# dusk-network/plonk_gadgets

Measured on AMD Instinct MI355X. Metric: gadget constraints/sec (range_check 256-bit), higher is better.
Workload: dtype u64x4 (BLS12-381 scalar, Montgomery limbs)

## Files before the change

### plonk_gadgets_amd/csrc/capi.hip

```cpp
#include "../../include/plonk_gadgets_hip.h"

#include <hip/hip_runtime.h>

#include <algorithm>
#include <cassert>
#include <cstdio>
#include <cstdlib>
#include <cstring>
#include <initializer_list>
#include <memory>
#include <new>
#include <functional>
#include <string>
#include <type_traits>
#include <utility>
#include <vector>

#include "emit.hpp"
#include "fr.hpp"
#include "range_gadgets.hpp"
#include "scalar_gadgets.hpp"
#include "composer.hpp"
#include "permutation.hpp"
#include "materialize.hpp"
// ... 191 lines not shown
#define PG_MIX_EARLY_TILES 1
#endif
#ifndef PG_INV_LANES_PER_CU
#define PG_INV_LANES_PER_CU 256
#endif
#ifndef PG_INV_MAX_PER_LANE
#define PG_INV_MAX_PER_LANE 32
#endif

pg_status launch_mix(pg_engine *e, const pg::ScalarMixArgs &A, const pg_columns *c, uint64_t batch, uint64_t gate_base,
                     uint64_t var_base, uint64_t zero_var, const uint64_t *row_off, const uint64_t *var_off, hipStream_t st,
                     const pg::MixPlan *planned, bool values_only = false) {
    using GD = pg::ScalarMixGD;
    PG_TRY(ensure_inv_scratch(e, batch));
    const uint64_t waves_wanted = (uint64_t)e->num_cus * 4 * 2;
    uint64_t ipl = (batch + waves_wanted * 32 - 1) / (waves_wanted * 32);
    if (ipl < 1) ipl = 1;
    if (ipl > pg::kMixMaxIpl) ipl = pg::kMixMaxIpl;
    const uint64_t waves = (batch + 32 * ipl - 1) / (32 * ipl);
    pg::EmitOut V = make_out(c, batch, GD::W, gate_base, var_base, zero_var, row_off, var_off);
    pg::EmitOut R = make_out(c, batch, GD::kRowsW, gate_base, var_base, zero_var, row_off, var_off);
    const uint64_t span = (uint64_t)pg::kMixWaves * 32 * ipl;
    if (!values_only && ipl >= 8 && span <= 0xffffffffull) {
        V.early_span = R.early_span = (uint32_t)span;
        V.early_tiles = R.early_tiles = PG_MIX_EARLY_TILES;
    }
    const uint32_t max_blocks = (uint32_t)e->num_cus * PG_GRID_BLOCKS_PER_CU;
    const dim3 grid(R.tiles < max_blocks ? R.tiles : max_blocks), vgrid((uint32_t)((waves + pg::kMixWaves - 1) / pg::kMixWaves));
    const dim3 vblock(pg::kMixWaves * 64);
    uint4 *const prefix = e->d_prefix.as<uint4>(), *sink = prefix + e->inv_elems * 4 + 4 * 32 * 32 * 8;
    if (planned) {
        pg::MixPlan P = *planned;
        P.nwaves = vgrid.x;
        hipLaunchKernelGGL(pg::scalar_mix_vars_kernel<true>, vgrid, vblock, 0, st, A, V, (uint32_t)ipl, prefix, sink, P);
    } else
        hipLaunchKernelGGL(pg::scalar_mix_vars_kernel<false>, vgrid, vblock, 0, st, A, V, (uint32_t)ipl, prefix, sink,
                           pg::MixPlan{});
    if (values_only) {
        PG_HIP_TRY(hipGetLastError());
        return PG_OK;
    }
    hipLaunchKernelGGL(pg::rows_periodic_kernel<GD>, grid, dim3(pg::kThreads), 0, st, A, R);
    hipLaunchKernelGGL((pg::emit_kernel<GD, pg::EMIT_ROWS>), grid, dim3(pg::kThreads), 0, st, A, R);
    PG_HIP_TRY(hipGetLastError());
    return PG_OK;
}

template <class GD> struct ValuesMode { static constexpr bool ok = !pg::Split<GD>::ok; };

template <class GD>
pg_status launch(pg_engine *e, const typename GD::Args &A, const pg_columns *c, uint64_t batch, uint64_t gate_base,
                 uint64_t var_base, uint64_t zero_var, const uint64_t *row_off, const uint64_t *var_off, void *stream,
                 const pg::MixPlan *planned = nullptr, bool values_only = false, uint32_t stride_rows = 0) {
    if ((batch + GD::W - 1) / GD::W > 0xffffffffull) return fail(PG_ERR_INVALID_ARGUMENT, "batch too large for one call");
    if (stride_rows && (batch > 0xffffffffull || pg::Split<GD>::ok || GD::kRagged))
        return fail(PG_ERR_INVALID_ARGUMENT, "a row stride is for uniform one-launch gadgets of at most 2^32 - 1 items");
    hipStream_t st = static_cast<hipStream_t>(stream);
    PG_TRY(enter_stream(e, st));
    StreamScope scope{e, st};
    if constexpr (pg::Split<GD>::ok) {
        return launch_mix(e, A, c, batch, gate_base, var_base, zero_var, row_off, var_off, st, planned, values_only);
    } else {
        pg::EmitOut O = make_out(c, batch, GD::W, gate_base, var_base, zero_var, row_off, var_off);
        if (stride_rows) {
            O.stride_rows = stride_rows;
            O.tiles = (uint32_t)batch;
        }
        bool side = false;
        SideJoin join{e, st};
        if constexpr (GD::kInv > 0) {
            constexpr int GRP = GD::kInvGroup;
            const uint64_t elems = batch * GD::kInv;
            PG_TRY(ensure_inv_scratch(e, elems));
            const uint64_t lanes_wanted = (uint64_t)e->num_cus * PG_INV_LANES_PER_CU;
            uint64_t per_lane = (elems + lanes_wanted - 1) / lanes_wanted;
            if (per_lane < 1) per_lane = 1;
            if (per_lane > PG_INV_MAX_PER_LANE) per_lane = PG_INV_MAX_PER_LANE;
            const uint64_t groups = (per_lane + GRP - 1) / GRP;
            const uint64_t lanes = (elems + groups * GRP - 1) / (groups * GRP);
            const uint32_t blocks = (uint32_t)((lanes + pg::kThreads - 1) / pg::kThreads);
            side = elems >= 2048 && elems < (1ull << 18);
            hipStream_t inv_st = st;
            if (side) {
                PG_HIP_TRY(hipEventRecord(e->ev_fork.get(), st));
                PG_HIP_TRY(hipStreamWaitEvent(e->side.get(), e->ev_fork.get(), 0));
                join.forked = true;
                inv_st = e->side.get();
            }
            if constexpr (pg::InvDense<GD>::ok) {
                O.inv_dense = e->d_prefix.as<uint4>();
                O.inv_elems = elems;
                O.inv_in_place = side;
            }
            hipLaunchKernelGGL((pg::batch_invert_kernel<GD, GRP>), dim3(blocks), dim3(pg::kThreads), 0, inv_st, A, O, elems,
                               (uint32_t)groups, e->d_prefix.as<uint4>());
            PG_HIP_TRY(hipGetLastError());
            if (side) PG_HIP_TRY(hipEventRecord(e->ev_inv.get(), e->side.get()));
        }
        const uint32_t max_blocks = (uint32_t)e->num_cus * (values_only ? PG_GRID_BLOCKS_PER_CU : PG_EMIT_GRID_BLOCKS_PER_CU);
        const dim3 egrid(O.tiles < max_blocks ? O.tiles : max_blocks);
        if (values_only) {
            if constexpr (ValuesMode<GD>::ok) hipLaunchKernelGGL((pg::emit_kernel<GD, pg::EMIT_VALUES>), egrid, dim3(pg::kThreads), 0, st, A, O);
            else return fail(PG_ERR_INVALID_ARGUMENT, "this gadget has no values-only emission");
        } else {
            hipLaunchKernelGGL(pg::emit_kernel<GD>, egrid, dim3(pg::kThreads), 0, st, A, O);
        }
        PG_HIP_TRY(hipGetLastError());
        if (side) {
            PG_HIP_TRY(hipStreamWaitEvent(st, e->ev_inv.get(), 0));
            join.joined = true;
        }
        return PG_OK;
    }
}

pg_status scalar_args(const pg_variable *a_var, const pg_scalar *a_val, const pg_variable *b_var,
// ... 1138 lines not shown
```

### plonk_gadgets_amd/csrc/emit.hpp

```cpp
#pragma once

#include <type_traits>

#include "fr.hpp"

namespace pg {

constexpr int kThreads = 256;

union FrVec {
    Fr f;
    uint4 v[2];
};

struct EmitOut {
    uint4 *q[5];
    uint64_t *w[3];
    uint4 *vars;
    uint64_t gate_base, var_base;
    uint64_t zero_var;
    const uint64_t *row_off;
    const uint64_t *var_off;
    uint64_t batch;
    uint32_t tiles;
    uint32_t stride_rows;
    const uint4 *inv_dense;
    uint64_t inv_elems;
    uint32_t inv_in_place;
    uint32_t early_span, early_tiles;
};
__device__ __forceinline__ bool early_rows_candidate(const EmitOut &O, uint64_t w0, uint32_t Wt, uint32_t W, uint64_t &s0, uint64_t &s1) {
    s0 = s1 = 0;
    if (!O.early_tiles || Wt != W) return false;
    s0 = w0 - w0 % O.early_span;
    s1 = s0 + O.early_span < O.batch ? s0 + O.early_span : O.batch;
    return (w0 - s0) / W < O.early_tiles;
}

__device__ __forceinline__ void fetch_inverse(const EmitOut &O, uint64_t s, void *rec_fr) {
    uint4 *z = reinterpret_cast<uint4 *>(rec_fr);
    z[0] = O.inv_dense[s];
    z[1] = O.inv_dense[O.inv_elems + s];
}

enum : uint32_t { T_ZERO = 0, T_ONE = 1, T_NEG1 = 2, T_QC_A = 3, T_QC_B = 4, T_POW = 8 };
constexpr int kTableEntries = 8 + 256;

typedef unsigned int pg_u32x4 __attribute__((ext_vector_type(4)));

__device__ __forceinline__ void store16(uint4 *p, uint4 v) {
#if defined(PG_NT_STORES)
    pg_u32x4 t = {v.x, v.y, v.z, v.w};
    __builtin_nontemporal_store(t, reinterpret_cast<pg_u32x4 *>(p));
#else
    *p = v;
#endif
}

__device__ __forceinline__ void lds_barrier() {
#if defined(PG_FULL_BARRIERS)
    __syncthreads();
#else
    asm volatile("s_waitcnt lgkmcnt(0)\n\ts_barrier" ::: "memory");
#endif
}

__device__ __forceinline__ uint64_t uniform64(uint64_t x) {
    return (uint64_t)(uint32_t)__builtin_amdgcn_readfirstlane((int)(uint32_t)x) |
           (uint64_t)(uint32_t)__builtin_amdgcn_readfirstlane((int)(uint32_t)(x >> 32)) << 32;
}

__device__ __forceinline__ Fr lds_fr(const uint4 *table, uint32_t id) {
    FrVec t;
    t.v[0] = table[2 * id];
    t.v[1] = table[2 * id + 1];
    return t.f;
}

__device__ __forceinline__ void fill_common_table(uint4 *table, const uint4 *pow2, uint32_t tid, uint32_t entries) {
    for (uint32_t e = tid; e < entries; e += kThreads) {
        FrVec t;
        t.f = fr_zero();
        if (e == T_ONE) t.f = fr_one();
        else if (e == T_NEG1) t.f = fr_neg_one();
        else if (e >= T_POW && pow2) { t.v[0] = pow2[(e - T_POW) * 2]; t.v[1] = pow2[(e - T_POW) * 2 + 1]; }
        if (e != T_QC_A && e != T_QC_B) {
            table[2 * e] = t.v[0];
            table[2 * e + 1] = t.v[1];
        }
    }
}

template <bool SMALL_ITEMS, uint32_t UNI>
__device__ __forceinline__ uint32_t find_item(const uint32_t *off, uint32_t Wt, uint32_t r, uint32_t it, bool uniform) {
    if constexpr (UNI != 0) {
        if (uniform) return r / UNI;
    }
    if constexpr (SMALL_ITEMS) {
// ... 22 lines not shown
struct Periodic {
    static constexpr bool ok = false;
};
template <class GD>
struct Periodic<GD, std::void_t<decltype(GD::kPeriodic)>> {
    static constexpr bool ok = GD::kPeriodic;
};
constexpr uint32_t periodic_wire_lanes(uint32_t R) {
    uint32_t L = 256;
    while ((2 * L) % R) L--;
    return L;
}

#ifndef PG_EMIT_WAVES_PER_SIMD
#define PG_EMIT_WAVES_PER_SIMD 1
#endif

enum EmitMode : int { EMIT_ALL = 0, EMIT_STRUCTURE = 1, EMIT_ROWS = 2, EMIT_VALUES = 3 };

template <class GD, class = void>
struct Split {
    static constexpr bool ok = false;
};
template <class GD>
struct Split<GD, std::void_t<decltype(GD::kSplit)>> {
    static constexpr bool ok = GD::kSplit;
};
template <class GD, class = void>
struct RegionVars {
    static constexpr bool ok = false;
};
template <class GD>
struct RegionVars<GD, std::void_t<decltype(GD::kRegionVars)>> {
    static constexpr bool ok = GD::kRegionVars;
};
template <class GD, class = void>
struct InvDense {
    static constexpr bool ok = false;
};
template <class GD>
struct InvDense<GD, std::void_t<decltype(GD::kInvDense)>> {
    static constexpr bool ok = GD::kInvDense;
};
template <class GD, int MODE>
struct EmitShape {
    using Rec = typename GD::ItemRec;
    static constexpr int W = GD::W;
};
template <class GD>
struct EmitShape<GD, EMIT_ROWS> {
    using Rec = typename GD::RowRec;
    static constexpr int W = GD::kRowsW;
};

constexpr uint32_t kRegionLead = 8, kRegionStage = (kRegionLead + 256 + 16) / 8 * 9;

template <class GD, int MODE = EMIT_ALL>
__global__ __launch_bounds__(kThreads, PG_EMIT_WAVES_PER_SIMD) void emit_kernel(const typename GD::Args A, const EmitOut O) {
    static_assert(MODE != EMIT_STRUCTURE || !(GD::kRagged || GD::kRecInRows), "rows of this gadget depend on its inputs");
    constexpr bool kVars = MODE == EMIT_ALL || MODE == EMIT_VALUES;
    constexpr bool kRows = MODE != EMIT_VALUES;
    constexpr int W = EmitShape<GD, MODE>::W;
    using Rec = typename EmitShape<GD, MODE>::Rec;
    constexpr uint32_t kTable = GD::kUsePow2 ? kTableEntries : T_POW;
    __shared__ uint4 s_table[kTable * 2];
    __shared__ Rec s_item[W];
    __shared__ uint32_t s_roff[W + 1], s_voff[W + 1];

    const uint32_t tid = threadIdx.x;
    {
        const uint4 *p2 = nullptr;
        if constexpr (GD::kUsePow2) p2 = GD::pow2(A);
        fill_common_table(s_table, p2, tid, kTable);
    }
    GD::fill_table(A, s_table, tid);
    lds_barrier();

    for (uint32_t t = blockIdx.x; t < O.tiles; t += gridDim.x) {
#if defined(PG_XCD_REMAP)
        const uint32_t q8 = O.tiles >> 3, r8 = O.tiles & 7, x = t & 7, k = t >> 3;
        const uint32_t tile = x * q8 + (x < r8 ? x : r8) + k;
#elif defined(PG_TILE_SPREAD)
        const uint32_t qs = O.tiles / PG_TILE_SPREAD, rs = O.tiles % PG_TILE_SPREAD, x = t % PG_TILE_SPREAD, k = t / PG_TILE_SPREAD;
        const uint32_t tile = x * qs + (x < rs ? x : rs) + k;
#else
        const uint32_t tile = t;
#endif
        const uint64_t w0 = O.stride_rows ? (uint64_t)tile : (uint64_t)tile * W;
        const uint32_t Wt = O.stride_rows ? 1u : (uint32_t)((O.batch - w0) < (uint64_t)W ? (O.batch - w0) : (uint64_t)W);
        if constexpr (MODE == EMIT_ROWS && Periodic<GD>::ok) {
            if (O.row_off[w0 + Wt] - O.row_off[w0] == (uint64_t)Wt * UniformShape<GD>::rows) continue;
        }
        uint64_t row0, var0;
        uint32_t G = 0, V = 0;
        uint64_t my_r = 0, my_v = 0, tail_r = 0, tail_v = 0;
        if constexpr (GD::kRagged) {
            row0 = O.row_off[w0];
            var0 = O.var_off[w0];
            if (tid <= Wt) {
                my_r = O.row_off[w0 + tid];
                my_v = O.var_off[w0 + tid];
            }
            if constexpr (W == kThreads) {
                if (tid == 0) {
                    tail_r = O.row_off[w0 + Wt];
                    tail_v = O.var_off[w0 + Wt];
                }
            }
        } else {
            G = GD::rows_per_item(A);
            V = GD::vars_per_item(A);
            row0 = w0 * (O.stride_rows ? O.stride_rows : G);
            var0 = w0 * V;
        }

        if constexpr ((GD::kRagged || GD::kRecInRows) && MODE != EMIT_STRUCTURE) {
            for (uint32_t i = tid; i < Wt; i += kThreads) GD::item_rows(A, O, w0 + i, s_table, s_item[i]);
        }
        if constexpr (GD::kRagged) {
            if (tid <= Wt) {
                s_roff[tid] = (uint32_t)(my_r - row0);
                s_voff[tid] = (uint32_t)(my_v - var0);
            }
            if constexpr (W == kThreads) {
                if (tid == 0) {
                    s_roff[Wt] = (uint32_t)(tail_r - row0);
                    s_voff[Wt] = (uint32_t)(tail_v - var0);
                }
            }
        }
        if constexpr (GD::kRagged || GD::kRecInRows) lds_barrier();
// ... 44 lines not shown
#if defined(PG_UNALIGNED_SWEEPS)
                const uint32_t pmis = 0;
#else
                const uint32_t pmis = (uint32_t)(((reinterpret_cast<uintptr_t>(col) - 8 * shift) >> 4) & 7u);
#endif
                uint32_t it = 0;
                for (uint32_t pv = tid < pmis ? tid + kThreads : tid; pv < pairs + pmis; pv += kThreads) {
                    const uint32_t p = pv - pmis;
                    const int64_t r0 = (int64_t)2 * p - shift;
                    uint64_t val[2];
#pragma unroll
                    for (int k = 0; k < 2; k++) {
                        const int64_t r = r0 + k;
                        uint32_t rr = r < 0 ? 0u : (uint32_t)r;
                        if (rr >= total_rows) rr = total_rows - 1;
                        uint32_t j, vo;
                        if constexpr (GD::kRagged) {
                            it = find_item<W >= 64, kUniR>(s_roff, Wt, rr, it, uni_rows);
                            j = uni_rows ? rr - it * kUniR : rr - s_roff[it];
                            vo = (uni_rows && uni_vars) ? it * kUniV : s_voff[it];
                        } else {
                            it = rr / G;
                            j = rr - it * G;
                            vo = it * V;
                        }
                        uint64_t out[3];
                        GD::wires(A, O, s_item[it], w0 + it, O.var_base + var0 + vo, j, out);
                        val[k] = out[c];
                    }
                    if (r0 >= 0 && r0 + 1 < (int64_t)total_rows) {
                        store16(reinterpret_cast<uint4 *>(col + r0),
                                make_uint4((uint32_t)val[0], (uint32_t)(val[0] >> 32), (uint32_t)val[1],
                                           (uint32_t)(val[1] >> 32)));
                    } else {
                        if (r0 >= 0) col[r0] = val[0];
                        if (r0 + 1 < (int64_t)total_rows) col[r0 + 1] = val[1];
                    }
                }
            }
        }

        lds_barrier();

        if constexpr (kVars) {
            const bool inv_here = InvDense<GD>::ok && !O.inv_in_place;
#if defined(PG_UNALIGNED_SWEEPS)
            const uint32_t smis = 0;
#else
            const uint32_t smis = (uint32_t)((reinterpret_cast<uintptr_t>(O.vars + var0 * 2) >> 5) & 3u);
#endif
#if !defined(PG_VAR_SWEEP_SINGLE)
            if constexpr (RegionVars<GD>::ok && MODE == EMIT_VALUES) {
                __shared__ uint4 s_reg[4 * kRegionStage];
                const uint32_t wave = tid >> 6, lane = tid & 63;
                uint4 *wp = s_reg + wave * kRegionStage;
                constexpr uint32_t B2 = 2 * GD::kBlocks;
                const uint32_t units = Wt * B2;
                const uint32_t tile_mis = (uint32_t)((reinterpret_cast<uintptr_t>(O.vars + var0 * 2) >> 5) & 3u);
                for (uint32_t q = wave; q < units; q += kThreads / 64) {
                    const uint32_t it = q / B2, r = q - it * B2, b = r >> 1;
                    const uint32_t kind = (r + (GD::kBlocks == 2 ? it : it >> 1)) & 1;
                    const Rec &R = s_item[it];
                    const auto &Bk = GD::region_block(R, b);
                    const uint32_t n = GD::region_n(A, R);
                    const uint32_t count = kind ? (n + 1 < 256 ? n + 1 : 256) : 256;
                    uint32_t vitem, vend;
                    if constexpr (GD::kRagged) {
                        vitem = uni_vars ? it * kUniV : s_voff[it];
                        vend = uni_vars ? vitem + kUniV : s_voff[it + 1];
                    } else {
                        vitem = it * V;
                        vend = vitem + V;
                    }
                    const uint32_t kfirst = GD::region_k(A, R, b, kind ? 257 : 1);
                    const uint32_t mis0 = (tile_mis + vitem) & 3u;
                    uint32_t ks, ke;
                    if (kind == 0) {
                        ks = b == 0 ? 0 : kfirst;
                        if (it != 0 || b != 0) ks += (4u - ((mis0 + ks) & 3u)) & 3u;
                        ke = kfirst + 256;
                        ke -= (mis0 + ke) & 3u;
                    } else {
                        ks = kfirst - ((mis0 + kfirst) & 3u);
                        ke = b + 1 < GD::kBlocks ? GD::region_k(A, R, b + 1, 1) : vend - vitem;
                        if (it + 1 != Wt || b + 1 < GD::kBlocks) ke += (4u - ((mis0 + ke) & 3u)) & 3u;
                    }
                    const uint32_t h_end = (count - 1) >> 7;
                    uint32_t hole = ~0u;
                    if (!inv_here)
                        for (uint32_t k = kfirst + count; k < ke && k < vend - vitem; k++)
                            if (GD::is_inv_slot(A, R, k)) hole = k;
                    FrVec v[4];
                    const uint32_t i0 = 4 * lane;
                    if (kind == 0) {
#pragma unroll
                        for (int t = 0; t < 4; t++) v[t].f = raw_bit(Bk.Tc, i0 + t) ? fr_one() : fr_zero();
                    } else {
                        v[0].f = fr_zero();
                        if (i0 && i0 < count) v[0].f = fr_to_mont(raw_low_bits(Bk.Tc, i0));
#pragma unroll
                        for (int t = 1; t < 4; t++) {
                            v[t].f = v[t - 1].f;
                            if (i0 + t < count && raw_bit(Bk.Tc, i0 + t - 1)) {
                                FrVec p;
                                p.v[0] = s_table[2 * (T_POW + i0 + t - 1)];
                                p.v[1] = s_table[2 * (T_POW + i0 + t - 1) + 1];
                                v[t].f = fr_add(v[t - 1].f, p.f);
                            }
                        }
                    }
                    const uint32_t npre = ks < kfirst ? kfirst - ks : 0, npost = ke > kfirst + count ? ke - (kfirst + count) : 0;
                    FrVec nb;
                    uint32_t nb_at = ~0u;
                    if (lane < npre + npost) {
                        const uint32_t k = lane < npre ? ks + lane : kfirst + count + (lane - npre);
                        const uint32_t vitem_n = vend - vitem;
                        nb.f = k < vitem_n ? GD::var_value(A, R, s_table, k) : GD::var_value(A, s_item[it + 1], s_table, k - vitem_n);
                        nb_at = kRegionLead + 2 * (k - kfirst) - (lane < npre ? 0 : 256 * h_end);
                    }
#pragma unroll
                    for (int h = 0; h < 2; h++) {
                        if ((lane >> 5) == (uint32_t)h) {
                            const uint32_t u0 = kRegionLead + 8 * (lane & 31), w0 = u0 + (u0 >> 3);
#pragma unroll
                            for (int t = 0; t < 4; t++) {
                                wp[w0 + 2 * t] = v[t].v[0];
                                wp[w0 + 2 * t + 1] = v[t].v[1];
                            }
                        }
                        if (h == 1 && lane == 31) {
#pragma unroll
                            for (int t = 0; t < 4; t++) {
                                wp[kRegionLead - 8 + 2 * t] = v[t].v[0];
                                wp[kRegionLead - 8 + 2 * t + 1] = v[t].v[1];
                            }
                        }
                        if (nb_at != ~0u && (lane < npre ? h == 0 : (uint32_t)h == h_end)) {
                            wp[nb_at + (nb_at >> 3)] = nb.v[0];
                            wp[nb_at + 1 + ((nb_at + 1) >> 3)] = nb.v[1];
                        }
                        asm volatile("" ::: "memory");
                        const uint32_t mid = kfirst + 128 - ((mis0 + kfirst + 128) & 3u);
                        const uint32_t lo = h == 0 ? ks : mid, hi = (uint32_t)h == h_end ? ke : (h == 0 ? mid : lo);
                        const uint32_t total = hi > lo ? 2 * (hi - lo) : 0;
                        uint4 *dst = O.vars + ((uint64_t)var0 + vitem + lo) * 2;
                        const uint32_t mis = (uint32_t)((reinterpret_cast<uintptr_t>(dst) >> 4) & 7u);
                        const uint32_t lead = kRegionLead + 2 * (lo - kfirst) - 256 * h;
#pragma unroll
                        for (int j = 0; j < 5; j++) {
                            const uint32_t g = 64 * j + lane - mis;
                            const uint32_t u = g + lead;
                            if (g < total && lo + (g >> 1) != hole) store16(dst + g, wp[u + (u >> 3)]);
                        }
                        asm volatile("" ::: "memory");
                    }
                }
            } else
#endif
            {
            const uint32_t sv0 = tid < smis ? tid + kThreads : tid;
                uint32_t it = 0, k = sv0 - smis;
                if constexpr (!GD::kRagged) { it = k / V; k -= it * V; }
                for (uint32_t sv = sv0; sv < total_vars + smis; sv += kThreads) {
                    const uint32_t s = sv - smis;
                    if constexpr (GD::kRagged) {
                        it = find_item<W >= 64, kUniV>(s_voff, Wt, s, it, uni_vars);
                        k = uni_vars ? s - it * kUniV : s - s_voff[it];
                    }
                    uint4 *dst = O.vars + (var0 + s) * 2;
                    if (inv_here || !GD::is_inv_slot(A, s_item[it], k)) {
// ... 396 lines not shown
```

### plonk_gadgets_amd/csrc/fr.hpp

```cpp
#pragma once

#include "experiment.hpp"

#include <stdint.h>

#if defined(__HIPCC__)
#include <hip/hip_runtime.h>
#define PG_HD __host__ __device__ __forceinline__
#else
#define PG_HD inline
#endif

namespace pg {

struct Fr {
    uint64_t l[4];
};

#define PG_Q0 0xffffffff00000001ull
#define PG_Q1 0x53bda402fffe5bfeull
#define PG_Q2 0x3339d80809a1d805ull
#define PG_Q3 0x73eda753299d7d48ull
#define PG_INV 0xfffffffeffffffffull

// ... 335 lines not shown
        b[2 * i] = (uint32_t)y.l[i]; b[2 * i + 1] = (uint32_t)(y.l[i] >> 32);
    }
    uint64_t acc = 0;
    uint32_t ex;
#pragma unroll
    for (int k = 0; k < 8; k++) {
        mac_run<true>(a, b, k, 0, k, acc, ex);
        if (k > 0) mac_run(m, Q, k, 0, k - 1, acc, ex);
        uint32_t nlo, nhi;
        asm("v_cmp_ne_u32 vcc, 0, %3\n\t"
            "v_sub_u32 %0, 0, %3\n\t"
            "s_nop 0\n\t"
            "v_addc_co_u32 %1, vcc, %4, 0, vcc\n\t"
            "s_nop 1\n\t"
            "v_addc_co_u32 %2, vcc, %5, 0, vcc\n\t"
            : "=&v"(m[k]), "=&v"(nlo), "=&v"(nhi)
            : "v"((uint32_t)acc), "v"((uint32_t)(acc >> 32)), "v"(ex)
            : "vcc");
        acc = (uint64_t)nlo | ((uint64_t)nhi << 32);
    }
#pragma unroll
    for (int k = 8; k < 15; k++) {
        mac_run<true>(a, b, k, k - 7, 7, acc, ex);
        mac_run(m, Q, k, k - 7, 7, acc, ex);
        r[k - 8] = (uint32_t)acc;
        acc = (acc >> 32) | ((uint64_t)ex << 32);
    }
    r[7] = (uint32_t)acc;
    return fr_final_sub_words(r, (uint32_t)(acc >> 32));
}
#else
PG_HD Fr fr_mul(const Fr &a, const Fr &b) { return fr_mul64(a, b); }
#endif

PG_HD Fr fr_square(const Fr &a) { return fr_mul(a, a); }

PG_HD Fr fr_to_mont(const Fr &raw) { return fr_mul(raw, fr_r2()); }
PG_HD Fr fr_from_mont(const Fr &a) {
    uint64_t t[8] = {a.l[0], a.l[1], a.l[2], a.l[3], 0, 0, 0, 0};
    return fr_mont_reduce(t);
}
PG_HD Fr fr_from_u64(uint64_t v) { return fr_to_mont(Fr{{v, 0, 0, 0}}); }

PG_HD uint32_t raw_bit(const Fr &c, uint32_t i) { return (uint32_t)(c.l[i >> 6] >> (i & 63)) & 1u; }
PG_HD Fr raw_low_bits(const Fr &c, uint32_t nbits) {
    Fr o;
    for (int i = 0; i < 4; i++) {
        uint32_t lo = 64u * i;
        uint64_t m = nbits >= lo + 64 ? ~0ull : (nbits <= lo ? 0ull : ((1ull << (nbits - lo)) - 1));
        o.l[i] = c.l[i] & m;
    }
    return o;
}
PG_HD bool raw_has_high_bits(const Fr &c, uint32_t nbits) {
    Fr lo = raw_low_bits(c, nbits);
    return !fr_eq(lo, c);
}
PG_HD uint32_t raw_bit_length(const Fr &c) {
    for (int i = 3; i >= 0; i--)
        if (c.l[i]) {
            uint32_t n = 0;
            uint64_t v = c.l[i];
            while (v) { n++; v >>= 1; }
            return 64u * i + n;
        }
    return 0;
}

PG_HD Fr fr_invert_fermat(const Fr &a) {
    const uint64_t E[4] = {0xfffffffeffffffffull, PG_Q1, PG_Q2, PG_Q3};
    Fr res = fr_one();
    bool started = false;
    for (int e = 3; e >= 0; e--) {
        for (int i = 63; i >= 0; i--) {
            if (started) res = fr_square(res);
            if ((E[e] >> i) & 1) {
                res = started ? fr_mul(res, a) : a;
                started = true;
            }
        }
    }
    return res;
}

struct Signed30 {
    int32_t v[9];
};
#define PG_M30 0x3fffffff
#define PG_Q30 {0x1, 0x3ffffffc, 0x3fe5bfef, 0x2f6900bf, 0x21d80553, 0x27602026, 0x17d48333, 0x29d4ca67, 0x73ed}

PG_HD void raw_to_signed30(const Fr &a, Signed30 &r) {
    r.v[0] = (int32_t)(a.l[0] & PG_M30);
    r.v[1] = (int32_t)((a.l[0] >> 30) & PG_M30);
    r.v[2] = (int32_t)(((a.l[0] >> 60) | (a.l[1] << 4)) & PG_M30);
    r.v[3] = (int32_t)((a.l[1] >> 26) & PG_M30);
    r.v[4] = (int32_t)(((a.l[1] >> 56) | (a.l[2] << 8)) & PG_M30);
    r.v[5] = (int32_t)((a.l[2] >> 22) & PG_M30);
    r.v[6] = (int32_t)(((a.l[2] >> 52) | (a.l[3] << 12)) & PG_M30);
    r.v[7] = (int32_t)((a.l[3] >> 18) & PG_M30);
    r.v[8] = (int32_t)(a.l[3] >> 48);
}
PG_HD Fr signed30_to_raw(const Signed30 &r) {
    const uint64_t v0 = (uint32_t)r.v[0], v1 = (uint32_t)r.v[1], v2 = (uint32_t)r.v[2], v3 = (uint32_t)r.v[3], v4 = (uint32_t)r.v[4],
                   v5 = (uint32_t)r.v[5], v6 = (uint32_t)r.v[6], v7 = (uint32_t)r.v[7], v8 = (uint32_t)r.v[8];
    return Fr{{v0 | v1 << 30 | v2 << 60, v2 >> 4 | v3 << 26 | v4 << 56, v4 >> 8 | v5 << 22 | v6 << 52, v6 >> 12 | v7 << 18 | v8 << 48}};
}
// ... 142 lines not shown
```

### plonk_gadgets_amd/csrc/range_gadgets.hpp

```cpp
#pragma once

#include "emit.hpp"
#include "invert.hpp"

namespace pg {

struct alignas(16) BoundRec {
    Fr Tm;
    Fr Tc;
    Fr UZ[2];
};

__device__ __forceinline__ void bound_fetch_z(const EmitOut &O, uint64_t s, BoundRec &b) { fetch_inverse(O, s, &b.UZ[1]); }

__device__ __forceinline__ Fr bound_u(const Fr &Tm, const Fr &Tc, uint32_t n) {
    if (!raw_has_high_bits(Tc, n)) return fr_zero();
    return fr_sub(fr_to_mont(raw_low_bits(Tc, n)), Tm);
}

__device__ __forceinline__ uint32_t bound_item(const Fr &Tm, uint32_t n, BoundRec &b) {
    const Fr Tc = fr_from_mont(Tm);
    b.Tm = Tm;
    b.Tc = Tc;
    const Fr u = bound_u(Tm, Tc, n);
// ... 4 lines not shown
__device__ __forceinline__ uint32_t bound_z_offset(uint32_t n) { return 259 + n; }

__device__ __forceinline__ void bound_selector_ids(uint32_t jj, uint32_t n, bool is_min, uint32_t id[5]) {
    uint32_t qm = T_ZERO, ql = T_ZERO, qr = T_ZERO, qo = T_NEG1, qc = T_ZERO;
    if (jj >= 2 && jj < 2 * n + 2) {
        if (jj & 1) {
            ql = T_POW + ((jj - 3) >> 1);
            qr = T_ONE;
        } else {
            qm = T_ONE;
        }
    } else if (jj == 0) {
        ql = is_min ? T_ONE : T_NEG1;
        qc = is_min ? T_QC_B : T_QC_A;
    } else if (jj == 1) {
        ql = T_ONE;
        qo = T_ZERO;
    } else if (jj == 2 * n + 2) {
        ql = T_ONE;
        qr = T_NEG1;
    } else if (jj == 2 * n + 3) {
        qm = T_NEG1;
        qc = T_ONE;
    } else {
        qm = T_ONE;
        qo = T_ZERO;
    }
    id[0] = qm; id[1] = ql; id[2] = qr; id[3] = qo; id[4] = qc;
}

constexpr uint32_t kWitnessWire = 0xffffffffu;

__device__ __forceinline__ void bound_wire_offsets(uint32_t jj, uint32_t n, uint32_t vb, uint32_t x, uint32_t off[3]) {
    uint32_t a, b, c;
    if (jj >= 2 && jj < 2 * n + 2) {
        const uint32_t i = (jj - 2) >> 1;
        a = vb + 1 + i;
        if (jj & 1) { b = vb + 257 + i; c = vb + 258 + i; }
        else { b = a; c = a; }
    } else if (jj == 0) {
        a = x; b = x; c = vb;
    } else if (jj == 1) {
        a = b = c = vb + 257;
    } else if (jj == 2 * n + 2) {
        a = vb + 257 + n; b = vb; c = vb + 258 + n;
    } else if (jj == 2 * n + 3) {
        a = vb + 259 + n; b = vb + 258 + n; c = vb + 260 + n;
    } else {
        a = vb + 260 + n; b = vb + 258 + n; c = b;
    }
    off[0] = a; off[1] = b; off[2] = c;
}

__device__ __forceinline__ Fr bound_var_value(const BoundRec &B, uint32_t y, uint32_t kk, uint32_t n) {
    if (kk == 0) return B.Tm;
    if (kk <= 256) return raw_bit(B.Tc, kk - 1) ? fr_one() : fr_zero();
    if (kk <= 257 + n) {
        const uint32_t i = kk - 257;
        return i ? fr_to_mont(raw_low_bits(B.Tc, i)) : fr_zero();
    }
    if (kk <= 259 + n) {
        const uint4 *p = reinterpret_cast<const uint4 *>(B.UZ) + 2 * (kk - (258 + n));
        FrVec v;
        v.v[0] = p[0];
        v.v[1] = p[1];
        return v.f;
    }
    return y ? fr_one() : fr_zero();
}

__device__ __forceinline__ void ids_to_values(const uint32_t id[5], const uint4 *table, uint32_t h, uint4 out[5]) {
#pragma unroll
    for (int c = 0; c < 5; c++) out[c] = table[2 * id[c] + h];
}

struct RangeCheckGD {
    struct Args {
        Fr min_range, max_range;
        uint32_t n;
        const uint4 *witness;
        const uint64_t *witness_vars;
        uint64_t *result_vars;
        const uint4 *pow2;
    };
    static constexpr int kInv = 2;
    static constexpr bool kInvDense = true;
    static constexpr int kInvGroup = 4;
    __device__ static void inv_operands(const Args &A, const EmitOut &, uint64_t item, uint32_t, FrVec &p, FrVec &q, uint32_t &) {
        p.v[0] = A.witness[item * 2];
        p.v[1] = A.witness[item * 2 + 1];
        q.f = p.f;
    }
    __device__ static Fr inv_combine(const Args &A, uint32_t e, const Fr &x, const Fr &, uint32_t) {
        const Fr t0 = fr_sub(fr_sub(A.max_range, fr_one()), x), t1 = fr_sub(x, A.min_range);
        Fr Tm;
#pragma unroll
        for (int i = 0; i < 4; i++) Tm.l[i] = e == 0 ? t0.l[i] : t1.l[i];
        return bound_u(Tm, fr_from_mont(Tm), A.n);
    }
    __device__ static uint4 *inv_slot(const Args &A, const EmitOut &O, uint64_t item, uint32_t e) {
        const uint64_t V = 2 * A.n + 523 + (A.witness_vars ? 0u : 1u), VB = A.n + 261;
        return O.vars + 2 * (item * V + (A.witness_vars ? 0u : 1u) + e * VB + bound_z_offset(A.n));
    }
    struct alignas(16) ItemRec {
        Fr x;
        BoundRec b[2];
        uint32_t y[2];
        uint32_t pad[2];
    };
    __device__ static bool is_inv_slot(const Args &A, const ItemRec &, uint32_t k) {
        const uint32_t x0 = A.witness_vars ? 0u : 1u, VB = A.n + 261, z = bound_z_offset(A.n);
        return k == x0 + z || k == x0 + VB + z;
    }
#ifndef PG_RC_W
#define PG_RC_W 32
#endif
    static constexpr int W = PG_RC_W;
    static constexpr bool kRagged = false, kRecInRows = false, kUsePow2 = true;

    __device__ static const uint4 *pow2(const Args &A) { return A.pow2; }
    __device__ static uint32_t rows_per_item(const Args &A) { return 4 * A.n + 11; }
    __device__ static uint32_t xo(const Args &A) { return A.witness_vars ? 0u : 1u; }
    __device__ static uint32_t vars_per_item(const Args &A) { return 2 * A.n + 523 + xo(A); }

    __device__ static void fill_table(const Args &A, uint4 *table, uint32_t tid) {
        if (tid == T_QC_A || tid == T_QC_B) {
            FrVec t;
            t.f = tid == T_QC_A ? fr_sub(A.max_range, fr_one())
                                : fr_neg(A.min_range);
            table[2 * tid] = t.v[0];
            table[2 * tid + 1] = t.v[1];
        }
    }

    __device__ static void item(const Args &A, const EmitOut &O, uint64_t item, const uint4 *table, ItemRec &R) {
        FrVec x;
        x.v[0] = A.witness[item * 2];
        x.v[1] = A.witness[item * 2 + 1];
        R.x = x.f;
        bound_fetch_z(O, item, R.b[0]);
        bound_fetch_z(O, O.batch + item, R.b[1]);
        R.y[0] = bound_item(fr_sub(lds_fr(table, T_QC_A), x.f), A.n, R.b[0]);
        R.y[1] = bound_item(fr_add(x.f, lds_fr(table, T_QC_B)), A.n, R.b[1]);
        const uint64_t V = vars_per_item(A);
        if (A.result_vars) A.result_vars[item] = O.var_base + item * V + (V - 1);
    }

    __device__ static void selectors(const Args &A, const ItemRec &, uint32_t j, const uint4 *table, uint32_t h, uint4 out[5]) {
        const uint32_t L = 2 * A.n + 5;
        uint32_t id[5];
        if (j == 2 * L) {
            id[0] = T_ONE; id[1] = T_ZERO; id[2] = T_ZERO; id[3] = T_NEG1; id[4] = T_ZERO;
        } else {
            const bool is_min = j >= L;
            bound_selector_ids(is_min ? j - L : j, A.n, is_min, id);
        }
        ids_to_values(id, table, h, out);
    }

    __device__ static void wires(const Args &A, const EmitOut &, const ItemRec &, uint64_t item, uint64_t vbase, uint32_t j,
                                 uint64_t out[3]) {
        const uint32_t n = A.n, L = 2 * n + 5, VB = n + 261, x0 = xo(A);
        uint32_t off[3];
        if (j == 2 * L) {
            off[0] = x0 + 260 + n;
            off[1] = x0 + VB + 260 + n;
            off[2] = x0 + 2 * VB;
        } else {
            const bool is_min = j >= L;
            bound_wire_offsets(is_min ? j - L : j, n, is_min ? x0 + VB : x0, kWitnessWire, off);
        }
        const uint64_t xvar = A.witness_vars ? A.witness_vars[item] : vbase;
#pragma unroll
        for (int c = 0; c < 3; c++) out[c] = off[c] == kWitnessWire ? xvar : vbase + off[c];
    }

    __device__ static Fr var_value(const Args &A, const ItemRec &R, const uint4 *, uint32_t k) {
        const uint32_t n = A.n, VB = n + 261;
        if (!A.witness_vars) {
            if (k == 0) return R.x;
            k -= 1;
        }
        if (k == 2 * VB) return (R.y[0] & R.y[1]) ? fr_one() : fr_zero();
        uint32_t kk = k, blk = 0;
        if (kk >= VB) { kk -= VB; blk = 1; }
        return bound_var_value(R.b[blk], R.y[blk], kk, n);
    }
    static constexpr bool kRegionVars = true;
    static constexpr uint32_t kBlocks = 2;
    __device__ static uint32_t region_n(const Args &A, const ItemRec &) { return A.n; }
    __device__ static const BoundRec &region_block(const ItemRec &R, uint32_t b) { return R.b[b]; }
    __device__ static uint32_t region_k(const Args &A, const ItemRec &, uint32_t b, uint32_t kk) { return xo(A) + b * (A.n + 261) + kk; }
};

template <bool RAGGED>
struct MaxBoundGD {
    struct Args {
        Fr max_range;
        uint32_t n;
        const uint4 *max_range_v;
        const uint32_t *num_bits_v;
        const uint4 *witness;
        const uint64_t *witness_vars;
        uint64_t *result_vars;
        const uint4 *pow2;
    };
    static constexpr int kInv = 1;
    static constexpr bool kInvDense = true;
    static constexpr int kInvGroup = 4;
    __device__ static uint4 *inv_slot(const Args &A, const EmitOut &O, uint64_t item, uint32_t) {
        const uint32_t n = RAGGED ? A.num_bits_v[item] : A.n;
        const uint32_t x0 = (!RAGGED && A.witness_vars) ? 0u : 1u;
        const uint64_t first = RAGGED ? O.var_off[item] : item * (uint64_t)(n + 261 + x0);
        return O.vars + 2 * (first + x0 + bound_z_offset(n));
    }
    __device__ static void inv_operands(const Args &A, const EmitOut &, uint64_t item, uint32_t, FrVec &p, FrVec &q, uint32_t &n) {
        p.v[0] = A.witness[item * 2];
        p.v[1] = A.witness[item * 2 + 1];
        n = A.n;
        q.f = A.max_range;
        if constexpr (RAGGED) {
            q.v[0] = A.max_range_v[item * 2];
            q.v[1] = A.max_range_v[item * 2 + 1];
            n = A.num_bits_v[item];
        }
    }
    __device__ static Fr inv_combine(const Args &, uint32_t, const Fr &x, const Fr &m, uint32_t n) {
        const Fr Tm = fr_sub(fr_sub(m, fr_one()), x);
        return bound_u(Tm, fr_from_mont(Tm), n);
    }
    struct alignas(16) ItemRec {
        Fr x;
        Fr qc;
        BoundRec b;
        uint32_t y, n;
        uint32_t pad[2];
    };
#ifndef PG_MB_W
#define PG_MB_W 16
// ... 25 lines not shown
        m.v[1] = A.max_range_v[item * 2 + 1];
        R.qc = fr_sub(m.f, fr_one());
        R.n = A.num_bits_v[item];
    }

    __device__ static void item(const Args &A, const EmitOut &O, uint64_t item, const uint4 *table, ItemRec &R) {
        FrVec x;
        x.v[0] = A.witness[item * 2];
        x.v[1] = A.witness[item * 2 + 1];
        R.x = x.f;
        bound_fetch_z(O, item, R.b);
        uint32_t n = A.n;
        Fr qc;
        if constexpr (RAGGED) {
            qc = R.qc;
            n = R.n;
        } else {
            qc = lds_fr(table, T_QC_A);
            R.qc = qc;
            R.n = n;
        }
        R.y = bound_item(fr_sub(qc, x.f), n, R.b);
        if (A.result_vars) {
            const uint64_t first = RAGGED ? O.var_off[item] : item * (uint64_t)(n + 261 + xo(A));
            A.result_vars[item] = O.var_base + first + (n + 260 + xo(A));
        }
    }

    __device__ static void selectors(const Args &A, const ItemRec &R, uint32_t j, const uint4 *table, uint32_t h, uint4 out[5]) {
        uint32_t id[5];
        bound_selector_ids(j, RAGGED ? R.n : A.n, false, id);
        ids_to_values(id, table, h, out);
        if constexpr (RAGGED) {
            if (j == 0) {
                FrVec q;
                q.f = R.qc;
                out[4] = q.v[h];
            }
        }
    }

    __device__ static void wires(const Args &A, const EmitOut &, const ItemRec &R, uint64_t item, uint64_t vbase, uint32_t j,
                                 uint64_t out[3]) {
        uint32_t off[3];
        bound_wire_offsets(j, RAGGED ? R.n : A.n, xo(A), kWitnessWire, off);
        const uint64_t xvar = xo(A) ? vbase : A.witness_vars[item];
#pragma unroll
        for (int c = 0; c < 3; c++) out[c] = off[c] == kWitnessWire ? xvar : vbase + off[c];
    }

    __device__ static bool is_inv_slot(const Args &A, const ItemRec &R, uint32_t k) {
        return k == xo(A) + bound_z_offset(RAGGED ? R.n : A.n);
    }
    __device__ static Fr var_value(const Args &A, const ItemRec &R, const uint4 *, uint32_t k) {
        if (xo(A)) {
            if (k == 0) return R.x;
            k -= 1;
        }
        return bound_var_value(R.b, R.y, k, RAGGED ? R.n : A.n);
    }
    static constexpr bool kRegionVars = true;
    static constexpr uint32_t kBlocks = 1;
    __device__ static uint32_t region_n(const Args &A, const ItemRec &R) { return RAGGED ? R.n : A.n; }
    __device__ static const BoundRec &region_block(const ItemRec &R, uint32_t) { return R.b; }
    __device__ static uint32_t region_k(const Args &A, const ItemRec &, uint32_t, uint32_t kk) { return xo(A) + kk; }
};

struct DecompositionGD {
    struct Args {
        uint32_t n;
        const uint4 *witness;
        const uint64_t *witness_vars;
        uint64_t *result_vars;
        const uint4 *pow2;
    };
    static constexpr int kInv = 1;
    static constexpr bool kInvDense = true;
    static constexpr int kInvGroup = 4;
    __device__ static void inv_operands(const Args &A, const EmitOut &, uint64_t item, uint32_t, FrVec &p, FrVec &q, uint32_t &) {
        p.v[0] = A.witness[item * 2];
        p.v[1] = A.witness[item * 2 + 1];
        q.f = p.f;
    }
    __device__ static Fr inv_combine(const Args &A, uint32_t, const Fr &x, const Fr &, uint32_t) {
        return bound_u(x, fr_from_mont(x), A.n);
    }
    __device__ static uint4 *inv_slot(const Args &A, const EmitOut &O, uint64_t item, uint32_t) {
        return O.vars + 2 * (item * (uint64_t)(A.n + 260) + bound_z_offset(A.n) - 1);
    }
    struct alignas(16) ItemRec {
        BoundRec b;
        uint32_t y, pad[3];
    };
    static constexpr int W = 32;
    static constexpr bool kRagged = false, kRecInRows = false, kUsePow2 = true;
    __device__ static const uint4 *pow2(const Args &A) { return A.pow2; }
    __device__ static uint32_t rows_per_item(const Args &A) { return 2 * A.n + 4; }
    __device__ static uint32_t vars_per_item(const Args &A) { return A.n + 260; }
    __device__ static void fill_table(const Args &, uint4 *table, uint32_t tid) {
        if (tid == T_QC_A || tid == T_QC_B) {
            table[2 * tid] = make_uint4(0, 0, 0, 0);
            table[2 * tid + 1] = make_uint4(0, 0, 0, 0);
        }
    }
    __device__ static void item(const Args &A, const EmitOut &O, uint64_t item, const uint4 *, ItemRec &R) {
        FrVec x;
        x.v[0] = A.witness[item * 2];
        x.v[1] = A.witness[item * 2 + 1];
        bound_fetch_z(O, item, R.b);
        R.y = bound_item(x.f, A.n, R.b);
        const uint64_t V = vars_per_item(A);
        if (A.result_vars) A.result_vars[item] = O.var_base + item * V + (V - 1);
    }
    __device__ static void selectors(const Args &A, const ItemRec &, uint32_t j, const uint4 *table, uint32_t h, uint4 out[5]) {
        uint32_t id[5];
        bound_selector_ids(j + 1, A.n, false, id);
        ids_to_values(id, table, h, out);
    }
    __device__ static void wires(const Args &A, const EmitOut &, const ItemRec &, uint64_t item, uint64_t vbase, uint32_t j,
                                 uint64_t out[3]) {
        uint32_t off[3];
        bound_wire_offsets(j + 1, A.n, kWitnessWire, kWitnessWire, off);
        const uint64_t xvar = A.witness_vars[item];
#pragma unroll
        for (int c = 0; c < 3; c++) out[c] = off[c] == kWitnessWire ? xvar : vbase + off[c];
    }
    __device__ static bool is_inv_slot(const Args &A, const ItemRec &, uint32_t k) { return k + 1 == bound_z_offset(A.n); }
    __device__ static Fr var_value(const Args &A, const ItemRec &R, const uint4 *, uint32_t k) {
        return bound_var_value(R.b, R.y, k + 1, A.n);
    }
    static constexpr bool kRegionVars = true;
    static constexpr uint32_t kBlocks = 1;
    __device__ static uint32_t region_n(const Args &A, const ItemRec &) { return A.n; }
    __device__ static const BoundRec &region_block(const ItemRec &R, uint32_t) { return R.b; }
    __device__ static uint32_t region_k(const Args &, const ItemRec &, uint32_t, uint32_t kk) { return kk - 1; }
};

__global__ __launch_bounds__(kThreads) void max_bound_plan_kernel(const uint4 *max_range, uint64_t batch, const uint4 *pow2,
                                                                 uint32_t *num_bits, uint32_t *rows, uint32_t *vars, const PlanScan P) {
    uint32_t r[4] = {0, 0, 0, 0}, v[4] = {0, 0, 0, 0};
#pragma unroll
    for (int k = 0; k < 4; k++) {
        const uint64_t i = (uint64_t)blockIdx.x * kScanBlock + threadIdx.x * 4 + k;
        if (i < batch) {
            FrVec m, p;
            m.v[0] = max_range[i * 2];
            m.v[1] = max_range[i * 2 + 1];
            const Fr mm1 = fr_sub(m.f, fr_one());
            uint32_t nb = raw_bit_length(fr_from_mont(mm1));
            if (nb < 1) nb = 1;
            p.v[0] = pow2[nb * 2];
            p.v[1] = pow2[nb * 2 + 1];
            uint32_t n = raw_bit_length(fr_from_mont(p.f));
            if (n < 1) n = 1;
            num_bits[i] = n;
            r[k] = 2 * n + 5;
            v[k] = n + 262;
        }
    }
    plan_store(P, r, v, batch, rows, vars);
}

__global__ void pow2_table_kernel(uint4 *out) {
    if (threadIdx.x != 0 || blockIdx.x != 0) return;
    FrVec p;
    p.f = fr_one();
    for (int i = 0; i < 256; i++) {
        out[2 * i] = p.v[0];
        out[2 * i + 1] = p.v[1];
        p.f = fr_add(p.f, p.f);
    }
}

}
```

Measured before the change: 32.67 billion.

## Compute running-sum values from per-word prefix sums instead of full to_mont

```diff
diff --git a/plonk_gadgets_amd/csrc/capi.hip b/plonk_gadgets_amd/csrc/capi.hip
--- a/plonk_gadgets_amd/csrc/capi.hip
+++ b/plonk_gadgets_amd/csrc/capi.hip
@@ -267,7 +267,8 @@
 pg_status launch(pg_engine *e, const typename GD::Args &A, const pg_columns *c, uint64_t batch, uint64_t gate_base,
                  uint64_t var_base, uint64_t zero_var, const uint64_t *row_off, const uint64_t *var_off, void *stream,
                  const pg::MixPlan *planned = nullptr, bool values_only = false, uint32_t stride_rows = 0) {
-    if ((batch + GD::W - 1) / GD::W > 0xffffffffull) return fail(PG_ERR_INVALID_ARGUMENT, "batch too large for one call");
+    const int W = values_only ? pg::EmitShape<GD, pg::EMIT_VALUES>::W : GD::W;
+    if ((batch + W - 1) / W > 0xffffffffull) return fail(PG_ERR_INVALID_ARGUMENT, "batch too large for one call");
     if (stride_rows && (batch > 0xffffffffull || pg::Split<GD>::ok || GD::kRagged))
         return fail(PG_ERR_INVALID_ARGUMENT, "a row stride is for uniform one-launch gadgets of at most 2^32 - 1 items");
     hipStream_t st = static_cast<hipStream_t>(stream);
@@ -276,7 +277,7 @@
     if constexpr (pg::Split<GD>::ok) {
         return launch_mix(e, A, c, batch, gate_base, var_base, zero_var, row_off, var_off, st, planned, values_only);
     } else {
-        pg::EmitOut O = make_out(c, batch, GD::W, gate_base, var_base, zero_var, row_off, var_off);
+        pg::EmitOut O = make_out(c, batch, W, gate_base, var_base, zero_var, row_off, var_off);
         if (stride_rows) {
             O.stride_rows = stride_rows;
             O.tiles = (uint32_t)batch;
diff --git a/plonk_gadgets_amd/csrc/emit.hpp b/plonk_gadgets_amd/csrc/emit.hpp
--- a/plonk_gadgets_amd/csrc/emit.hpp
+++ b/plonk_gadgets_amd/csrc/emit.hpp
@@ -43,7 +43,7 @@
     z[1] = O.inv_dense[O.inv_elems + s];
 }
 
-enum : uint32_t { T_ZERO = 0, T_ONE = 1, T_NEG1 = 2, T_QC_A = 3, T_QC_B = 4, T_POW = 8 };
+enum : uint32_t { T_ZERO = 0, T_ONE = 1, T_NEG1 = 2, T_QC_A = 3, T_QC_B = 4, T_R2 = 5, T_POW = 8 };
 constexpr int kTableEntries = 8 + 256;
 
 typedef unsigned int pg_u32x4 __attribute__((ext_vector_type(4)));
@@ -172,11 +172,26 @@
     using Rec = typename GD::RowRec;
     static constexpr int W = GD::kRowsW;
 };
+template <class GD, class = void>
+struct ValuesW {
+    static constexpr int W = GD::W;
+};
+template <class GD>
+struct ValuesW<GD, std::void_t<decltype(GD::kValuesW)>> {
+    static constexpr int W = GD::kValuesW;
+};
+template <class GD>
+struct EmitShape<GD, EMIT_VALUES> {
+    using Rec = typename GD::ItemRec;
+    static constexpr int W = ValuesW<GD>::W;
+};
 
 constexpr uint32_t kRegionLead = 8, kRegionStage = (kRegionLead + 256 + 16) / 8 * 9;
+constexpr uint32_t kRegionWords = 7;
 
 template <class GD, int MODE = EMIT_ALL>
-__global__ __launch_bounds__(kThreads, PG_EMIT_WAVES_PER_SIMD) void emit_kernel(const typename GD::Args A, const EmitOut O) {
+__global__ __launch_bounds__(kThreads, (RegionVars<GD>::ok && MODE == EMIT_VALUES) ? 4 : PG_EMIT_WAVES_PER_SIMD) void emit_kernel(
+    const typename GD::Args A, const EmitOut O) {
     static_assert(MODE != EMIT_STRUCTURE || !(GD::kRagged || GD::kRecInRows), "rows of this gadget depend on its inputs");
     constexpr bool kVars = MODE == EMIT_ALL || MODE == EMIT_VALUES;
     constexpr bool kRows = MODE != EMIT_VALUES;
@@ -194,9 +209,20 @@
         fill_common_table(s_table, p2, tid, kTable);
     }
     GD::fill_table(A, s_table, tid);
+    if constexpr (RegionVars<GD>::ok && MODE == EMIT_VALUES) {
+        if (tid == T_R2) {
+            FrVec t;
+            t.f = fr_r2();
+            s_table[2 * T_R2] = t.v[0];
+            s_table[2 * T_R2 + 1] = t.v[1];
+        }
+    }
     lds_barrier();
 
+    const uint32_t tid_wg = tid;
     for (uint32_t t = blockIdx.x; t < O.tiles; t += gridDim.x) {
+        uint32_t tid = tid_wg;
+        if constexpr (RegionVars<GD>::ok && MODE == EMIT_VALUES) asm volatile("" : "+v"(tid));
 #if defined(PG_XCD_REMAP)
         const uint32_t q8 = O.tiles >> 3, r8 = O.tiles & 7, x = t & 7, k = t >> 3;
         const uint32_t tile = x * q8 + (x < r8 ? x : r8) + k;
@@ -347,6 +373,28 @@
 #if !defined(PG_VAR_SWEEP_SINGLE)
             if constexpr (RegionVars<GD>::ok && MODE == EMIT_VALUES) {
                 __shared__ uint4 s_reg[4 * kRegionStage];
+                __shared__ uint4 s_pref[W * GD::kBlocks * kRegionWords * 2];
+                for (uint32_t p = tid; p < Wt * GD::kBlocks * kRegionWords; p += kThreads) {
+                    const uint32_t ib = p / kRegionWords, a = p - ib * kRegionWords;
+                    const auto &Bp = GD::region_block(s_item[ib / GD::kBlocks], ib % GD::kBlocks);
+                    FrVec x;
+                    x.f = fr_redc1_mul_u32(raw_word(Bp.Tc, a), lds_fr(s_table, T_POW + 32 * (a + 1)));
+                    s_pref[2 * p] = x.v[0];
+                    s_pref[2 * p + 1] = x.v[1];
+                }
+                lds_barrier();
+                if (tid < Wt * GD::kBlocks) {
+                    uint4 *pp = s_pref + 2 * kRegionWords * tid;
+                    Fr acc = lds_fr(pp, 0);
+                    for (uint32_t a = 1; a < kRegionWords; a++) {
+                        FrVec x;
+                        x.f = fr_add(acc, lds_fr(pp, a));
+                        pp[2 * a] = x.v[0];
+                        pp[2 * a + 1] = x.v[1];
+                        acc = x.f;
+                    }
+                }
+                lds_barrier();
                 const uint32_t wave = tid >> 6, lane = tid & 63;
                 uint4 *wp = s_reg + wave * kRegionStage;
                 constexpr uint32_t B2 = 2 * GD::kBlocks;
@@ -391,8 +439,11 @@
 #pragma unroll
                         for (int t = 0; t < 4; t++) v[t].f = raw_bit(Bk.Tc, i0 + t) ? fr_one() : fr_zero();
                     } else {
-                        v[0].f = fr_zero();
-                        if (i0 && i0 < count) v[0].f = fr_to_mont(raw_low_bits(Bk.Tc, i0));
+                        const uint32_t a = lane >> 3;
+                        FrVec P;
+                        P.f = lds_fr(s_pref, (it * GD::kBlocks + b) * kRegionWords + (a ? a - 1 : 0));
+                        if (!a) P.f = fr_zero();
+                        v[0].f = fr_low_bits_from_prefix(Bk.Tc, i0, P.f, lds_fr(s_table, a < 7 ? T_POW + 32 * (a + 1) : T_R2));
 #pragma unroll
                         for (int t = 1; t < 4; t++) {
                             v[t].f = v[t - 1].f;
@@ -410,7 +461,8 @@
                     if (lane < npre + npost) {
                         const uint32_t k = lane < npre ? ks + lane : kfirst + count + (lane - npre);
                         const uint32_t vitem_n = vend - vitem;
-                        nb.f = k < vitem_n ? GD::var_value(A, R, s_table, k) : GD::var_value(A, s_item[it + 1], s_table, k - vitem_n);
+                        const Rec &Rn = k < vitem_n ? R : s_item[it + 1];
+                        nb.f = GD::template var_value<false>(A, Rn, s_table, k < vitem_n ? k : k - vitem_n);
                         nb_at = kRegionLead + 2 * (k - kfirst) - (lane < npre ? 0 : 256 * h_end);
                     }
 #pragma unroll
diff --git a/plonk_gadgets_amd/csrc/fr.hpp b/plonk_gadgets_amd/csrc/fr.hpp
--- a/plonk_gadgets_amd/csrc/fr.hpp
+++ b/plonk_gadgets_amd/csrc/fr.hpp
@@ -411,6 +411,45 @@
     }
     return o;
 }
+PG_HD uint32_t raw_word(const Fr &c, uint32_t a) { return (uint32_t)(c.l[a >> 1] >> (32u * (a & 1u))); }
+
+PG_HD Fr fr_redc1_mul_u32(uint32_t w, const Fr &X) {
+    const uint32_t Q[8] = {0x00000001u, 0xffffffffu, 0xfffe5bfeu, 0x53bda402u, 0x09a1d805u, 0x3339d808u, 0x299d7d48u, 0x73eda753u};
+    uint32_t t[9], r[8];
+    uint64_t c = 0;
+#if defined(__HIP_DEVICE_COMPILE__)
+#pragma unroll
+#endif
+    for (int i = 0; i < 8; i++) {
+        c += (uint64_t)w * raw_word(X, (uint32_t)i);
+        t[i] = (uint32_t)c;
+        c >>= 32;
+    }
+    t[8] = (uint32_t)c;
+    const uint32_t m = 0u - t[0];
+    c = ((uint64_t)t[0] + m) >> 32;
+#if defined(__HIP_DEVICE_COMPILE__)
+#pragma unroll
+#endif
+    for (int i = 1; i < 8; i++) {
+        c += (uint64_t)t[i] + (uint64_t)m * Q[i];
+        r[i - 1] = (uint32_t)c;
+        c >>= 32;
+    }
+    r[7] = (uint32_t)(c + t[8]);
+#if defined(__HIP_DEVICE_COMPILE__)
+    return fr_final_sub_words(r, 0);
+#else
+    const uint64_t r64[4] = {r[0] | (uint64_t)r[1] << 32, r[2] | (uint64_t)r[3] << 32, r[4] | (uint64_t)r[5] << 32, r[6] | (uint64_t)r[7] << 32};
+    return fr_final_sub(r64, 0);
+#endif
+}
+
+PG_HD Fr fr_low_bits_from_prefix(const Fr &Tc, uint32_t i, const Fr &P, const Fr &X) {
+    const uint32_t w = raw_word(Tc, i >> 5) & ((1u << (i & 31u)) - 1u);
+    return fr_add(P, fr_redc1_mul_u32(w, X));
+}
+
 PG_HD bool raw_has_high_bits(const Fr &c, uint32_t nbits) {
     Fr lo = raw_low_bits(c, nbits);
     return !fr_eq(lo, c);
diff --git a/plonk_gadgets_amd/csrc/range_gadgets.hpp b/plonk_gadgets_amd/csrc/range_gadgets.hpp
--- a/plonk_gadgets_amd/csrc/range_gadgets.hpp
+++ b/plonk_gadgets_amd/csrc/range_gadgets.hpp
@@ -80,10 +80,12 @@
     off[0] = a; off[1] = b; off[2] = c;
 }
 
+template <bool RUNS = true>
 __device__ __forceinline__ Fr bound_var_value(const BoundRec &B, uint32_t y, uint32_t kk, uint32_t n) {
     if (kk == 0) return B.Tm;
     if (kk <= 256) return raw_bit(B.Tc, kk - 1) ? fr_one() : fr_zero();
     if (kk <= 257 + n) {
+        if constexpr (!RUNS) return B.Tm;
         const uint32_t i = kk - 257;
         return i ? fr_to_mont(raw_low_bits(B.Tc, i)) : fr_zero();
     }
@@ -144,6 +146,7 @@
 #define PG_RC_W 32
 #endif
     static constexpr int W = PG_RC_W;
+    static constexpr int kValuesW = W < 16 ? W : 16;
     static constexpr bool kRagged = false, kRecInRows = false, kUsePow2 = true;
 
     __device__ static const uint4 *pow2(const Args &A) { return A.pow2; }
@@ -203,6 +206,7 @@
         for (int c = 0; c < 3; c++) out[c] = off[c] == kWitnessWire ? xvar : vbase + off[c];
     }
 
+    template <bool RUNS = true>
     __device__ static Fr var_value(const Args &A, const ItemRec &R, const uint4 *, uint32_t k) {
         const uint32_t n = A.n, VB = n + 261;
         if (!A.witness_vars) {
@@ -212,7 +216,7 @@
         if (k == 2 * VB) return (R.y[0] & R.y[1]) ? fr_one() : fr_zero();
         uint32_t kk = k, blk = 0;
         if (kk >= VB) { kk -= VB; blk = 1; }
-        return bound_var_value(R.b[blk], R.y[blk], kk, n);
+        return bound_var_value<RUNS>(R.b[blk], R.y[blk], kk, n);
     }
     static constexpr bool kRegionVars = true;
     static constexpr uint32_t kBlocks = 2;
@@ -344,12 +348,13 @@
     __device__ static bool is_inv_slot(const Args &A, const ItemRec &R, uint32_t k) {
         return k == xo(A) + bound_z_offset(RAGGED ? R.n : A.n);
     }
+    template <bool RUNS = true>
     __device__ static Fr var_value(const Args &A, const ItemRec &R, const uint4 *, uint32_t k) {
         if (xo(A)) {
             if (k == 0) return R.x;
             k -= 1;
         }
-        return bound_var_value(R.b, R.y, k, RAGGED ? R.n : A.n);
+        return bound_var_value<RUNS>(R.b, R.y, k, RAGGED ? R.n : A.n);
     }
     static constexpr bool kRegionVars = true;
     static constexpr uint32_t kBlocks = 1;
@@ -418,8 +423,9 @@
         for (int c = 0; c < 3; c++) out[c] = off[c] == kWitnessWire ? xvar : vbase + off[c];
     }
     __device__ static bool is_inv_slot(const Args &A, const ItemRec &, uint32_t k) { return k + 1 == bound_z_offset(A.n); }
+    template <bool RUNS = true>
     __device__ static Fr var_value(const Args &A, const ItemRec &R, const uint4 *, uint32_t k) {
-        return bound_var_value(R.b, R.y, k + 1, A.n);
+        return bound_var_value<RUNS>(R.b, R.y, k + 1, A.n);
     }
     static constexpr bool kRegionVars = true;
     static constexpr uint32_t kBlocks = 1;
```

Result: no change. 32.62 billion (-0.2%).
